# bupt-cist/vqa-playground-pytorch

Measured on AMD Instinct MI355X. Metric: VQA samples/sec (fwd+bwd), CoR2 batch 512, 36x2048 regions, higher is better.
Workload: dtype f32

## Files before the change

### vqa_playground_pytorch_amd/csrc/gemm_f32_split.hpp

```cpp
#pragma once
#include <type_traits>

#include "gemm_f32_rt.hpp"

namespace vqa {
namespace sp {

using rt::f32x4;
using rt::ldg16;
using rt::make_rsrc;
using rt::rsrc_t;
typedef uint32_t u32x4 __attribute__((ext_vector_type(4)));

constexpr int kThreads = 256;
constexpr int kChunk = 32;
constexpr int kPackedChunkBytes = 3 * 1024;

typedef float f32x2 __attribute__((ext_vector_type(2)));
typedef __bf16 bf16x2 __attribute__((ext_vector_type(2)));
__device__ __forceinline__ uint32_t opaque(uint32_t v) {
  asm("" : "+v"(v));
  return v;
}
__device__ __forceinline__ uint32_t pack2(f32x2 v) { return __builtin_bit_cast(uint32_t, __builtin_convertvector(v, bf16x2)); }
template <bool DOT>
__device__ __forceinline__ f32x2 residual(f32x2 x, uint32_t p) {
  if constexpr (DOT) {
    const bf16x2 pv = __builtin_bit_cast(bf16x2, p);
    const bf16x2 m0 = __builtin_bit_cast(bf16x2, opaque(0x0000BF80u)), m1 = __builtin_bit_cast(bf16x2, opaque(0xBF800000u));
    return f32x2{__builtin_amdgcn_fdot2_f32_bf16(pv, m0, x[0], false), __builtin_amdgcn_fdot2_f32_bf16(pv, m1, x[1], false)};
  } else {
    const f32x2 w = {bf16_lo(p), bf16_hi(p)};
    return x - w;
  }
}
template <bool DOT>
__device__ __forceinline__ void split_pair(f32x2 x, uint32_t& p0, uint32_t& p1, uint32_t& p2) {
  p0 = opaque(pack2(x));
  const f32x2 r = residual<DOT>(x, p0);
  p1 = opaque(pack2(r));
  const f32x2 t = residual<DOT>(r, p1);
  p2 = pack2(t);
}
struct Planes {
  u32x4 p[3];
};
template <bool DOT = true>
__device__ __forceinline__ void split8(const f32x4& lo, const f32x4& hi, Planes& o) {
  uint32_t w[3][4];
  split_pair<DOT>(__builtin_shufflevector(lo, lo, 0, 1), w[0][0], w[1][0], w[2][0]);
  split_pair<DOT>(__builtin_shufflevector(lo, lo, 2, 3), w[0][1], w[1][1], w[2][1]);
  split_pair<DOT>(__builtin_shufflevector(hi, hi, 0, 1), w[0][2], w[1][2], w[2][2]);
  split_pair<DOT>(__builtin_shufflevector(hi, hi, 2, 3), w[0][3], w[1][3], w[2][3]);
#pragma unroll
  for (int q = 0; q < 3; ++q) o.p[q] = u32x4{w[q][0], w[q][1], w[q][2], w[q][3]};
}
__device__ __forceinline__ f32x4 mfma_bf16(const u32x4& a, const u32x4& b, const f32x4& c) {
  return __builtin_amdgcn_mfma_f32_16x16x32_bf16(__builtin_bit_cast(bf16x8, a), __builtin_bit_cast(bf16x8, b), c, 0, 0, 0);
}

__device__ __forceinline__ uint32_t abs_bits_max(const f32x4& v) {
  const u32x4 b = __builtin_bit_cast(u32x4, v) & 0x7FFFFFFFu;
  return max(max(b[0], b[1]), max(b[2], b[3]));
}
__device__ __forceinline__ bool any_nonfinite(const f32x4& v) { return abs_bits_max(v) >= 0x7F800000u; }
__device__ __forceinline__ bool nonfinite(float v) { return (__float_as_uint(v) & 0x7FFFFFFFu) >= 0x7F800000u; }

template <bool DOT = false>
__global__ __launch_bounds__(256) void split_pack_kernel(const float* __restrict__ w, int ldw, int N, int K,
                                                         u32x4* __restrict__ out) {
  const int chunks = K / kChunk;
  const long t = (long)blockIdx.x * 256 + threadIdx.x;
  const int nblocks = (N + 15) / 16;
  if (t >= (long)nblocks * chunks * 64) return;
  const int lane = (int)(t & 63), r = lane & 15, g = lane >> 4;
  const long bc = t >> 6;
  const int c = (int)(bc % chunks), n = (int)(bc / chunks) * 16 + r;
  f32x4 lo = f32x4{0.f, 0.f, 0.f, 0.f}, hi = lo;
  if (n < N) {
    const float* src = w + (size_t)n * ldw + c * kChunk + 4 * g;
    lo = *reinterpret_cast<const f32x4*>(src);
    hi = *reinterpret_cast<const f32x4*>(src + 16);
  }
  Planes pl;
  split8<DOT>(lo, hi, pl);
  u32x4* dst = out + (size_t)bc * 192 + lane;
  dst[0] = pl.p[0];
  dst[64] = pl.p[1];
  dst[128] = pl.p[2];
}
__host__ __device__ inline size_t packed_bytes(int N, int K) { return (size_t)((N + 15) / 16) * (K / kChunk) * kPackedChunkBytes; }

struct NtArgs {
  const float* A;
  const u32x4* Bp;
  int lda;
  int M, N, K;
  int tiles_n;
  const float* Bf = nullptr;
  int ldb = 0;
  const float* T = nullptr;
  const float* C2 = nullptr;
  int rps = 0;
};
__host__ __device__ inline int rel_samples(int BM, int rps) { return (BM - 1) / rps + 2; }
__host__ __device__ inline size_t rel_lds_bytes(int BM, int rps, int K) { return (size_t)rel_samples(BM, rps) * 2 * K * 4; }
template <bool DROP>
__device__ __forceinline__ float nt_repair(const float* A, int lda, const float* Bf, int ldb, int K, int row, int col, uint32_t key,
                                           const float* T = nullptr, const float* C2 = nullptr, int rps = 1) {
  const float* a = A + (size_t)row * lda;
  const float* b = Bf + (size_t)col * ldb;
  float s = 0.f;
  for (int k = 0; k < K; ++k) {
    float x = a[k];
    if (T != nullptr) x = fmaf(C2[(size_t)(row / rps) * K + k], x, T[(size_t)(row / rps) * K + k]);
    if constexpr (DROP) {
      const uint32_t e = (uint32_t)row * (uint32_t)K + (uint32_t)k;
      x = ((mask_word32(e >> 5, key) >> (e & 31u)) & 1u) != 0u ? x : 0.f;
    }
    s = fmaf(x, b[k], s);
  }
  return s;
}

template <int RB, int CB, bool DROP, int TUNE, int NR, bool REL = false>
__device__ __forceinline__ void nt_accumulate(const NtArgs& p, const DropCfg& dc, size_t a_bytes, int m0, int n0, int c_lo, int c_hi,
                                              f32x4 (&acc)[RB][CB], const char* rel_lds = nullptr, int rel_s0 = 0) {
  static_assert((2 * RB) % NR == 0 && NR >= 2 && NR <= 2 * RB, "the ring must divide a pair of chunks");
  const int lane = threadIdx.x & 63, r = lane & 15, g = lane >> 4;
  const int chunks = p.K / kChunk;
  uint32_t offA[RB], offB[CB], wordA[RB];
  uint32_t offT[REL ? RB : 1];
#pragma unroll
  for (int i = 0; i < RB; ++i) {
    const int row = min(m0 + 16 * i + r, p.M - 1);
    offA[i] = ((uint32_t)row * (uint32_t)p.lda + 4u * g) * 4u;
    wordA[i] = ((uint32_t)row * (uint32_t)p.K) >> 5;
    if constexpr (REL) offT[i] = ((uint32_t)(row / p.rps - rel_s0) * 2u * (uint32_t)p.K + 4u * g) * 4u;
  }
#pragma unroll
  for (int j = 0; j < CB; ++j) {
    const int blk = min((n0 >> 4) + j, (p.N + 15) / 16 - 1);
    offB[j] = (uint32_t)blk * (uint32_t)chunks * (uint32_t)kPackedChunkBytes + 16u * lane;
  }
  const rsrc_t Ab = make_rsrc(p.A, a_bytes);
  const rsrc_t Bb = make_rsrc(p.Bp, packed_bytes(p.N, p.K));
  const uint32_t key = DROP ? drop_key(dc) : 0u;

  struct ARaw {
    f32x4 lo, hi;
  };
  auto loadA = [&](ARaw& a, int i, int c) {
    const uint32_t so = (uint32_t)c * 128u;
    constexpr int AUX = (TUNE & 128) ? 2 : 0;
    a.lo = __builtin_bit_cast(f32x4, __builtin_amdgcn_raw_buffer_load_b128(Ab, (int)offA[i], (int)so, AUX));
    a.hi = __builtin_bit_cast(f32x4, __builtin_amdgcn_raw_buffer_load_b128(Ab, (int)(offA[i] + 64u), (int)so, AUX));
  };
  auto loadB = [&](Planes(&b)[CB], int c) {
    const uint32_t so = (uint32_t)c * (uint32_t)kPackedChunkBytes;
#pragma unroll
    for (int j = 0; j < CB; ++j)
#pragma unroll
      for (int q = 0; q < 3; ++q)
        b[j].p[q] = __builtin_bit_cast(u32x4, __builtin_amdgcn_raw_buffer_load_b128(Bb, (int)(offB[j] + 1024u * q), (int)so, 0));
  };
  struct TC {
    f32x4 tlo, thi, clo, chi;
  };
  TC tc[REL ? 2 : 1];
  auto loadTC = [&](TC& o, int i, int c) {
    if constexpr (REL) {
      const char* base = rel_lds + offT[i] + (uint32_t)c * 128u;
      o.tlo = *reinterpret_cast<const f32x4*>(base);
      o.thi = *reinterpret_cast<const f32x4*>(base + 64);
      o.clo = *reinterpret_cast<const f32x4*>(base + (size_t)p.K * 4);
      o.chi = *reinterpret_cast<const f32x4*>(base + (size_t)p.K * 4 + 64);
    }
  };
  auto prepare = [&](const ARaw& a, Planes& pl, int i, int c, int n = 0) {
    if constexpr ((TUNE & 1) != 0) {
      pl.p[0] = __builtin_bit_cast(u32x4, a.lo);
      pl.p[1] = __builtin_bit_cast(u32x4, a.hi);
      pl.p[2] = __builtin_bit_cast(u32x4, a.lo);
    } else {
      ARaw m = a;
      if constexpr (REL) {
        const TC& q = tc[n & 1];
        m.lo = __builtin_elementwise_fma(q.clo, m.lo, q.tlo);
        m.hi = __builtin_elementwise_fma(q.chi, m.hi, q.thi);
      }
      if constexpr (DROP) {
        const uint32_t w = mask_word32(wordA[i] + (uint32_t)c, key);
        rt::keep4_bits(m.lo, w >> (4u * g));
        rt::keep4_bits(m.hi, w >> (4u * g + 16u));
      }
      split8<(TUNE & 64) != 0>(m.lo, m.hi, pl);
    }
  };
  auto mfma_row = [&](const Planes& a, const Planes(&b)[CB], int i) {
    constexpr int PA[6] = {0, 0, 1, 1, 0, 2}, PB[6] = {0, 1, 0, 1, 2, 0};
#pragma unroll
    for (int q = 0; q < 6; ++q)
#pragma unroll
      for (int j = 0; j < CB; ++j) acc[i][j] = mfma_bf16(a.p[PA[q]], b[j].p[PB[q]], acc[i][j]);
  };

  ARaw a[NR];
  Planes b0[CB], b1[CB], pl[2];
  auto fetch = [&](int n, int c_pair) {
    const int c = min(c_pair + n / RB, c_hi - 1);
    loadA(a[n % NR], n % RB, c);
  };
  auto loadB1 = [&](Planes(&b)[CB], int idx, int c) {
    b[idx / 3].p[idx % 3] = __builtin_bit_cast(u32x4, __builtin_amdgcn_raw_buffer_load_b128(
        Bb, (int)(offB[idx / 3] + 1024u * (idx % 3)), (int)((uint32_t)c * (uint32_t)kPackedChunkBytes), 0));
  };
  auto chunk = [&](Planes(&b)[CB], Planes(&bn)[CB], int c_pair, auto parity) {
    constexpr int P = decltype(parity)::value;
    constexpr int LB = (3 * CB + RB - 1) / RB;
    const int cb = min(c_pair + P + 1, c_hi - 1);
#pragma unroll
    for (int i = 0; i < RB; ++i) {
      const int n = P * RB + i;
      prepare(a[(n + 1) % NR], pl[(n + 1) & 1], (n + 1) % RB, min(c_pair + (n + 1) / RB, c_hi - 1), n + 1);
      if constexpr (REL) loadTC(tc[n & 1], (n + 2) % RB, min(c_pair + (n + 2) / RB, c_hi - 1));
      if constexpr ((TUNE & 2) == 0) fetch(n + 1 + NR, c_pair);
      int nb = 0;
      if constexpr ((TUNE & 32) == 0) {
#pragma unroll
        for (int idx = i * LB; idx < (i + 1) * LB && idx < 3 * CB; ++idx, ++nb) loadB1(bn, idx, cb);
      }
      mfma_row(pl[n & 1], b, i);
      constexpr int NM = 6 * CB;
      constexpr int VPM = ((TUNE >> 2) & 3) != 0 ? ((TUNE >> 2) & 3) : 2;
      const int nl = nb + ((TUNE & 2) == 0 ? 2 : 0);
      const int per = nl > 0 ? NM / nl : NM;
#pragma unroll
      for (int m = 0; m < NM; ++m) {
        __builtin_amdgcn_sched_group_barrier(0x008, 1, 0);
        if (REL && m < 4) __builtin_amdgcn_sched_group_barrier(0x100, 1, 0);
        __builtin_amdgcn_sched_group_barrier(0x002, VPM, 0);
        if (nl > 0 && m % per == per - 1 && m / per < nl) __builtin_amdgcn_sched_group_barrier(0x020, 1, 0);
      }
      __builtin_amdgcn_sched_barrier(0);
    }
  };
  if (c_lo < c_hi) {
    loadB(b0, c_lo);
#pragma unroll
    for (int n = 0; n < NR; ++n) fetch(n, c_lo);
    if constexpr (REL) {
      loadTC(tc[0], 0, c_lo);
      loadTC(tc[1], 1 % RB, min(c_lo + 1 / RB, c_hi - 1));
    }
    prepare(a[0], pl[0], 0, c_lo, 0);
    fetch(NR, c_lo);
    __builtin_amdgcn_sched_barrier(0);
    for (int c = c_lo; c < c_hi; c += 2) {
      chunk(b0, b1, c, std::integral_constant<int, 0>{});
      chunk(b1, b0, c, std::integral_constant<int, 1>{});
    }
  }

}

template <int RB, int CB, int NW, bool DROP, int TUNE>
__device__ __forceinline__ void nt_accumulate_shared(const NtArgs& p, const DropCfg& dc, size_t a_bytes, int m0, int n0, int c_lo,
                                                     int c_hi, int wave, char* lds_bytes, f32x4 (&acc)[RB][CB]) {
  constexpr int MINE = (RB + NW - 1) / NW;
  const int lane = threadIdx.x & 63, r = lane & 15, g = lane >> 4;
  const int chunks = p.K / kChunk;
  u32x4* const lds = reinterpret_cast<u32x4*>(lds_bytes);
  uint32_t offA[MINE], offB[CB], wordA[MINE];
#pragma unroll
  for (int k = 0; k < MINE; ++k) {
    const int i = min(wave + NW * k, RB - 1);
    const int row = min(m0 + 16 * i + r, p.M - 1);
    offA[k] = ((uint32_t)row * (uint32_t)p.lda + 4u * g) * 4u;
    wordA[k] = ((uint32_t)row * (uint32_t)p.K) >> 5;
  }
  const uint32_t key = DROP ? drop_key(dc) : 0u;
#pragma unroll
  for (int j = 0; j < CB; ++j) {
    const int blk = min((n0 >> 4) + j, (p.N + 15) / 16 - 1);
    offB[j] = (uint32_t)blk * (uint32_t)chunks * (uint32_t)kPackedChunkBytes + 16u * lane;
  }
  const rsrc_t Ab = make_rsrc(p.A, a_bytes);
  const rsrc_t Bb = make_rsrc(p.Bp, packed_bytes(p.N, p.K));
  struct ARaw {
    f32x4 lo, hi;
  };
  ARaw raw0[MINE], raw1[MINE];
  Planes b0[CB], b1[CB], xp[2];
  auto loadA = [&](ARaw(&raw)[MINE], int c) {
    const uint32_t so = (uint32_t)min(c, c_hi - 1) * 128u;
#pragma unroll
    for (int k = 0; k < MINE; ++k) {
      raw[k].lo = ldg16(Ab, offA[k], so);
      raw[k].hi = ldg16(Ab, offA[k] + 64u, so);
    }
  };
  auto loadB1 = [&](Planes(&b)[CB], int idx, int c) {
    b[idx / 3].p[idx % 3] = __builtin_bit_cast(u32x4, __builtin_amdgcn_raw_buffer_load_b128(
        Bb, (int)(offB[idx / 3] + 1024u * (idx % 3)), (int)((uint32_t)min(c, c_hi - 1) * (uint32_t)kPackedChunkBytes), 0));
  };
  auto produce = [&](const ARaw& a, int k, int buf, int c) {
    if (wave + NW * k < RB) {
      Planes pl;
      ARaw m = a;
      if constexpr (DROP) {
        const uint32_t w = mask_word32(wordA[k] + (uint32_t)min(c, c_hi - 1), key);
        rt::keep4_bits(m.lo, w >> (4u * g));
        rt::keep4_bits(m.hi, w >> (4u * g + 16u));
      }
      split8<false>(m.lo, m.hi, pl);
      u32x4* dst = lds + ((size_t)(buf * RB + wave + NW * k) * 3) * 64 + lane;
#pragma unroll
      for (int q = 0; q < 3; ++q) dst[64 * q] = pl.p[q];
    }
  };
  auto fetch = [&](Planes& o, int i, int buf) {
    const u32x4* src = lds + ((size_t)(buf * RB + i) * 3) * 64 + lane;
#pragma unroll
    for (int q = 0; q < 3; ++q) o.p[q] = src[64 * q];
  };
  auto mfma_row = [&](const Planes& a, const Planes(&b)[CB], int i) {
    constexpr int PA[6] = {0, 0, 1, 1, 0, 2}, PB[6] = {0, 1, 0, 1, 2, 0};
#pragma unroll
    for (int q = 0; q < 6; ++q)
#pragma unroll
      for (int j = 0; j < CB; ++j) acc[i][j] = mfma_bf16(a.p[PA[q]], b[j].p[PB[q]], acc[i][j]);
  };
  auto chunk = [&](Planes(&b)[CB], Planes(&bn)[CB], ARaw(&rn)[MINE], ARaw(&rf)[MINE], int c, auto parity) {
    constexpr int P = decltype(parity)::value;
    constexpr int LB = (3 * CB + RB - 2) / (RB - 1);
    int bidx = 0, pk = 0;
#pragma unroll
    for (int i = 0; i < RB; ++i) {
      const int n = P * RB + i;
      if (i == RB - 1) __syncthreads();
      if (i + 1 < RB) fetch(xp[(n + 1) & 1], i + 1, P);
      else fetch(xp[(n + 1) & 1], 0, P ^ 1);
      if (i == 0) loadA(rf, c + 2);
      if (i >= 1 && pk < MINE && i < RB - 1) {
        produce(rn[pk], pk, P ^ 1, c + 1);
        ++pk;
      }
      int nl = 0;
      if (i < RB - 1) {
#pragma unroll
        for (int k = 0; k < LB; ++k)
          if (bidx < 3 * CB) {
            loadB1(bn, bidx, c + 1);
            ++bidx;
            ++nl;
          }
      }
      mfma_row(xp[n & 1], b, i);
      constexpr int NM = 6 * CB;
#pragma unroll
      for (int m = 0; m < NM; ++m) {
        __builtin_amdgcn_sched_group_barrier(0x008, 1, 0);
        if (m < 3) __builtin_amdgcn_sched_group_barrier(0x100, 1, 0);
        __builtin_amdgcn_sched_group_barrier(0x002, 2, 0);
        if (m >= 4 && m < 4 + 2 * (2 * MINE + LB) && (m & 1) == 0) __builtin_amdgcn_sched_group_barrier(0x020, 1, 0);
        if (m >= NM - 6 && (m & 1) == 0) __builtin_amdgcn_sched_group_barrier(0x200, 1, 0);
      }
      __builtin_amdgcn_sched_barrier(0);
    }
  };
  static_assert(MINE <= RB - 2, "a wave's row blocks are produced in the regions 1 .. RB - 2");
  if (c_lo < c_hi) {
#pragma unroll
    for (int idx = 0; idx < 3 * CB; ++idx) loadB1(b0, idx, c_lo);
    loadA(raw0, c_lo);
    loadA(raw1, c_lo + 1);
#pragma unroll
    for (int k = 0; k < MINE; ++k) produce(raw0[k], k, 0, c_lo);
    __syncthreads();
    fetch(xp[0], 0, 0);
    __builtin_amdgcn_sched_barrier(0);
    for (int c = c_lo; c < c_hi; c += 2) {
      chunk(b0, b1, raw1, raw0, c, std::integral_constant<int, 0>{});
      chunk(b1, b0, raw0, raw1, c + 1, std::integral_constant<int, 1>{});
    }
  }
}

template <int RB, int WN, int WK, bool SHARE_A>
constexpr size_t nt_lds_bytes(size_t reduction_bytes) {
  return SHARE_A ? (reduction_bytes > (size_t)WK * 2 * RB * 3 * 1024 ? reduction_bytes : (size_t)WK * 2 * RB * 3 * 1024) : reduction_bytes;
}
template <int RB, int CB, int WM, int WN, int WK, bool DROP, class Epi, int TUNE = 0, int NR = RB, bool SHARE_A = false, bool REL = false>
__global__ __launch_bounds__(kThreads, 1) void gemm_nt_kernel(NtArgs p, DropCfg dc, Epi epi) {
  using S = rt::NtShape<RB, CB, WM, WN, WK>;
  static_assert(!SHARE_A || WM == 1, "SHARE_A: the waves of a K range share their rows");
  static_assert(!(REL && SHARE_A), "REL is built on the per-wave split");
  const int lane = threadIdx.x & 63, r = lane & 15, g = lane >> 4;
  const int wave = __builtin_amdgcn_readfirstlane(threadIdx.x >> 6);
  const int wk = wave / (WM * WN), wmn = wave % (WM * WN), wm = wmn / WN, wn = wmn % WN;
  const int tile = xcd_remap(blockIdx.x, gridDim.x);
  const int tiles_m = gridDim.x / p.tiles_n;
  const int tm = (TUNE & 16) ? tile % tiles_m : tile / p.tiles_n, tn = (TUNE & 16) ? tile / tiles_m : tile % p.tiles_n;
  const int m0 = tm * S::BM + wm * (16 * RB);
  const int n0 = tn * S::BN + wn * (16 * CB);
  const int chunks = p.K / kChunk;

  f32x4 acc[RB][CB];
#pragma unroll
  for (int i = 0; i < RB; ++i)
#pragma unroll
    for (int j = 0; j < CB; ++j) acc[i][j] = f32x4{0.f, 0.f, 0.f, 0.f};
  const int per = ((chunks + WK - 1) / WK + 1) & ~1;
  const int c_lo = min(chunks, wk * per), c_hi = min(chunks, c_lo + per);

  if constexpr (SHARE_A) {
    extern __shared__ __attribute__((aligned(16))) char sp_smem[];
    nt_accumulate_shared<RB, CB, WN, DROP, TUNE>(p, dc, ((size_t)(p.M - 1) * p.lda + p.K) * 4, m0, n0, c_lo, c_hi, wn,
                                                 sp_smem + (size_t)wk * 2 * RB * 3 * 1024, acc);
    __syncthreads();
  } else if constexpr (REL) {
    extern __shared__ __attribute__((aligned(16))) char sp_smem[];
    const int s0 = (tm * S::BM) / p.rps;
    const int ns = (min(p.M, (tm + 1) * S::BM) - 1) / p.rps - s0 + 1;
    const int k4 = p.K / 4;
    const int total = ns * 2 * k4, iters = (total + kThreads - 1) / kThreads;
    for (int it = 0; it < iters; ++it) {
      const int idx = min(it * kThreads + (int)threadIdx.x, total - 1);
      const int s = idx / (2 * k4), rem = idx - s * 2 * k4, which = rem / k4, k = rem - which * k4;
      const float* src = (which == 0 ? p.T : p.C2) + (size_t)(s0 + s) * p.K + 4 * k;
      reinterpret_cast<f32x4*>(sp_smem)[idx] = *reinterpret_cast<const f32x4*>(src);
    }
    __syncthreads();
    nt_accumulate<RB, CB, DROP, TUNE, NR, true>(p, dc, ((size_t)(p.M - 1) * p.lda + p.K) * 4, m0, n0, c_lo, c_hi, acc, sp_smem, s0);
    __syncthreads();
  } else {
    nt_accumulate<RB, CB, DROP, TUNE, NR>(p, dc, ((size_t)(p.M - 1) * p.lda + p.K) * 4, m0, n0, c_lo, c_hi, acc);
  }

  uint64_t bad = 0;
  auto finish = [&](int blk, f32x4 v) {
    const int i = blk / CB, j = blk % CB;
    const int col = n0 + 16 * j + r;
    if (any_nonfinite(v)) bad |= 1ull << blk;
    if (col < p.N) {
#pragma unroll
      for (int t = 0; t < 4; ++t) {
        const int row = m0 + 16 * i + 4 * g + t;
        if (row < p.M) epi(row, col, v[t]);
      }
    }
  };
  if constexpr (WK == 2) {
    extern __shared__ __attribute__((aligned(16))) char sp_smem[];
    f32x4* red = reinterpret_cast<f32x4*>(sp_smem);
    f32x4* out_box = red + (size_t)((wmn * 2 + wk) * S::HALF) * 64 + lane;
    const f32x4* in_box = red + (size_t)((wmn * 2 + (wk ^ 1)) * S::HALF) * 64 + lane;
    if (wk == 0) {
#pragma unroll
      for (int blk = S::HALF; blk < S::NB; ++blk) out_box[(blk - S::HALF) * 64] = acc[blk / CB][blk % CB];
    } else {
#pragma unroll
      for (int blk = 0; blk < S::HALF; ++blk) out_box[blk * 64] = acc[blk / CB][blk % CB];
    }
    __syncthreads();
    if (wk == 0) {
#pragma unroll
      for (int blk = 0; blk < S::HALF; ++blk) finish(blk, acc[blk / CB][blk % CB] + in_box[blk * 64]);
    } else {
#pragma unroll
      for (int blk = S::HALF; blk < S::NB; ++blk) finish(blk, acc[blk / CB][blk % CB] + in_box[(blk - S::HALF) * 64]);
    }
  } else {
#pragma unroll
    for (int blk = 0; blk < S::NB; ++blk) finish(blk, acc[blk / CB][blk % CB]);
  }
  static_assert(S::NB <= 64, "one bit per accumulator block");
  if (p.Bf != nullptr && bad != 0) {
    const uint32_t key = DROP ? drop_key(dc) : 0u;
    for (int blk = 0; blk < S::NB; ++blk) {
      if (((bad >> blk) & 1ull) == 0) continue;
      const int col = n0 + 16 * (blk % CB) + r;
      if (col >= p.N) continue;
      for (int t = 0; t < 4; ++t) {
        const int row = m0 + 16 * (blk / CB) + 4 * g + t;
        if (row < p.M) epi(row, col, nt_repair<DROP>(p.A, p.lda, p.Bf, p.ldb, p.K, row, col, key, REL ? p.T : nullptr, p.C2, REL ? p.rps : 1));
      }
    }
  }
}


struct TnArgs {
  const u32x4* Gp;
  const float* X;
  float* slab;
  int ldx;
  int M, N1, N2;
  int nblocks;
  int cps;
  int tiles1, tiles2;
  const float* Gf = nullptr;
  const float* Yf = nullptr;
  int ldg = 0;
  const float* T = nullptr;
  const float* C2 = nullptr;
  int rps = 0;
  uint32_t rps_magic = 0;
};
inline uint32_t rps_magic_of(int rps) { return (uint32_t)((1ull << 32) / (uint64_t)rps + 1ull); }
template <int NA, int SPN, bool DROP>
__device__ __forceinline__ void tn_store(const TnArgs& p, const DropCfg& dc, const f32x4 (&acc)[NA][4 * SPN], int slab, int b1, int n2_0,
                                         int r, int g) {
  float* out = p.slab + (size_t)slab * p.N1 * p.N2;
  uint64_t bad = 0;
  static_assert(NA * SPN * 4 <= 64, "one bit per 16-byte store");
#pragma unroll
  for (int i = 0; i < NA; ++i)
#pragma unroll
    for (int q = 0; q < SPN; ++q) {
      const int col = n2_0 + 64 * q + 4 * r;
#pragma unroll
      for (int t = 0; t < 4; ++t) {
        const int n1 = 16 * (b1 + i) + 4 * g + t;
        const f32x4 v = f32x4{acc[i][4 * q][t], acc[i][4 * q + 1][t], acc[i][4 * q + 2][t], acc[i][4 * q + 3][t]};
        if (b1 + i < p.nblocks && n1 < p.N1 && col + 3 < p.N2) {
          *reinterpret_cast<f32x4*>(out + (size_t)n1 * p.N2 + col) = v;
          if (any_nonfinite(v)) bad |= 1ull << ((i * SPN + q) * 4 + t);
        }
      }
    }
  if (p.Gf != nullptr && bad != 0) {
    const uint32_t key = DROP ? drop_key(dc) : 0u;
    const int m_lo = slab * p.cps * kChunk, m_hi = min(p.M, m_lo + p.cps * kChunk);
    for (int k = 0; k < NA * SPN * 4; ++k) {
      if (((bad >> k) & 1ull) == 0) continue;
      const int t = k & 3, q = (k >> 2) % SPN, i = (k >> 2) / SPN;
      const int n1 = 16 * (b1 + i) + 4 * g + t, col = n2_0 + 64 * q + 4 * r;
      f32x4 sum = f32x4{0.f, 0.f, 0.f, 0.f};
      for (int m = m_lo; m < m_hi; ++m) {
        float gv = p.Gf[(size_t)m * p.ldg + n1];
        if (p.Yf != nullptr) gv = p.Yf[(size_t)m * p.ldg + n1] > 0.f ? gv : 0.f;
        f32x4 x = *reinterpret_cast<const f32x4*>(p.X + (size_t)m * p.ldx + col);
        if (p.T != nullptr) {
          const size_t at = (size_t)(m / p.rps) * p.N2 + col;
          x = __builtin_elementwise_fma(*reinterpret_cast<const f32x4*>(p.C2 + at), x, *reinterpret_cast<const f32x4*>(p.T + at));
        }
        if constexpr (DROP) {
          const uint32_t e = (uint32_t)m * (uint32_t)p.N2 + (uint32_t)col;
          const uint32_t w = mask_word32(e >> 5, key) >> (e & 31u);
#pragma unroll
          for (int c = 0; c < 4; ++c) x[c] = ((w >> c) & 1u) != 0u ? x[c] : 0.f;
        }
#pragma unroll
        for (int c = 0; c < 4; ++c) sum[c] = fmaf(gv, x[c], sum[c]);
      }
      *reinterpret_cast<f32x4*>(out + (size_t)n1 * p.N2 + col) = sum;
    }
  }
}
struct TnPlan {
  int slabs, cps;
};
inline TnPlan tn_plan(int M, int want_slabs) {
  const int chunks = (M + kChunk - 1) / kChunk;
  int S = want_slabs < 1 ? 1 : want_slabs;
  if (S > (chunks + 1) / 2) S = (chunks + 1) / 2;
  int cps = ((chunks + S - 1) / S + 1) & ~1;
  S = (chunks + cps - 1) / cps;
  return {S, cps};
}
__host__ __device__ inline size_t packed_tn_bytes(int slabs, int cps, int N1) {
  return (size_t)slabs * cps * ((N1 + 15) / 16) * kPackedChunkBytes;
}

constexpr int kPackParts = 36;
template <bool GATE, bool WRITE_GZ>
__global__ __launch_bounds__(256) void pack_tn_kernel(const float* __restrict__ gy, const float* __restrict__ y, int ld, int M,
                                                      int N1_all, int nblocks, int cps, u32x4* __restrict__ out,
                                                      float* __restrict__ dbslab, float* __restrict__ gz, int nblk_total) {
  extern __shared__ __attribute__((aligned(16))) float pk_tile[];
  const int pitch = 16 * nblocks + 1;
  const int lane = threadIdx.x & 63, r = lane & 15, g = lane >> 4, wave = threadIdx.x >> 6;
  const int slab = blockIdx.x / kPackParts, part = blockIdx.x % kPackParts;
  const int per = (cps + kPackParts - 1) / kPackParts;
  const int lo = part * per, hi = min(cps, lo + per);
  const int blk0 = blockIdx.y * nblocks, c0 = 16 * blk0;
  const int N1 = min(N1_all - c0, 16 * nblocks);
  gy += c0;
  if (GATE) y += c0;
  if (WRITE_GZ) gz += c0;
  const int pairs = N1 / 2;
  float colsum[8];
#pragma unroll
  for (int k = 0; k < 8; ++k) colsum[k] = 0.f;
  for (int cc = lo; cc < hi; ++cc) {
    const int c = slab * cps + cc;
    const int m0 = c * kChunk;
#pragma unroll 2
    for (int row = wave; row < 32; row += 4) {
      const int m = m0 + row;
      for (int cp = lane; cp < pairs; cp += 64) {
        float2 v = make_float2(0.f, 0.f);
        if (m < M) {
          v = *reinterpret_cast<const float2*>(gy + (size_t)m * ld + 2 * cp);
          if constexpr (GATE) {
            const float2 yy = *reinterpret_cast<const float2*>(y + (size_t)m * ld + 2 * cp);
            v.x = yy.x > 0.f ? v.x : 0.f;
            v.y = yy.y > 0.f ? v.y : 0.f;
          }
          if constexpr (WRITE_GZ) *reinterpret_cast<float2*>(gz + (size_t)m * ld + 2 * cp) = v;
        }
        pk_tile[row * pitch + 2 * cp] = v.x;
        pk_tile[row * pitch + 2 * cp + 1] = v.y;
      }
    }
    __syncthreads();
#pragma unroll
    for (int k = 0; k < 8; ++k) {
      const int blk = wave + 4 * k;
      if (blk < nblocks && blk0 + blk < nblk_total) {
        const int col = 16 * blk + r;
        float v[8];
#pragma unroll
        for (int j = 0; j < 8; ++j) v[j] = col < N1 ? pk_tile[(8 * g + j) * pitch + col] : 0.f;
        uint32_t w[3][4];
#pragma unroll
        for (int jj = 0; jj < 4; ++jj) {
          split_pair<false>(f32x2{v[2 * jj], v[2 * jj + 1]}, w[0][jj], w[1][jj], w[2][jj]);
          colsum[k] += v[2 * jj] + v[2 * jj + 1];
        }
        u32x4* dst = out + ((size_t)c * nblk_total + blk0 + blk) * 192 + lane;
#pragma unroll
        for (int q = 0; q < 3; ++q) dst[64 * q] = u32x4{w[q][0], w[q][1], w[q][2], w[q][3]};
      }
    }
    __syncthreads();
  }
  if (dbslab != nullptr) {
#pragma unroll
    for (int k = 0; k < 8; ++k) {
      float sum = colsum[k];
      sum += __shfl_xor(sum, 16);
      sum += __shfl_xor(sum, 32);
      const int col = 16 * (wave + 4 * k) + r;
      if (g == 0 && wave + 4 * k < nblocks && col < N1) dbslab[(size_t)blockIdx.x * N1_all + c0 + col] = sum;
    }
  }
}
inline size_t pack_tn_lds_bytes(int nblocks) { return (size_t)32 * (16 * nblocks + 1) * sizeof(float); }
constexpr int kPackMaxBlocks = 30;

template <int NA, int SPN, bool DROP, int TUNE = 0>
__global__ __launch_bounds__(kThreads, 1) void gemm_tn_kernel(TnArgs p, DropCfg dc) {
  constexpr int NBX = 4 * SPN;
  static_assert(NBX % 2 == 0, "plane sets alternate per block");
  const int lane = threadIdx.x & 63, r = lane & 15, g = lane >> 4;
  const int wave = __builtin_amdgcn_readfirstlane(threadIdx.x >> 6);
  const int bid = xcd_remap(blockIdx.x, gridDim.x);
  const int tiles = p.tiles1 * p.tiles2;
  const int slab = bid / tiles, tile = bid % tiles;
  const int t2 = tile % p.tiles2, t1 = tile / p.tiles2;
  const int b1 = (t1 * 4 + wave) * NA;
  const int n2_0 = t2 * (64 * SPN);
  const int c_lo = slab * p.cps, c_hi = c_lo + p.cps;

  uint32_t offX[8], offG[NA];
#pragma unroll
  for (int j = 0; j < 8; ++j)
    offX[j] = ((uint32_t)(8 * g + j) * (uint32_t)p.ldx + (uint32_t)min(n2_0 + 4 * r, p.N2 - 4)) * 4u;
#pragma unroll
  for (int i = 0; i < NA; ++i) offG[i] = (uint32_t)min(b1 + i, p.nblocks - 1) * (uint32_t)kPackedChunkBytes + 16u * lane;
  const rsrc_t Xb = make_rsrc(p.X, ((size_t)(p.M - 1) * p.ldx + p.N2) * 4);
  const rsrc_t Gb = make_rsrc(p.Gp, (size_t)gridDim.x / tiles * p.cps * p.nblocks * kPackedChunkBytes);
  const uint32_t key = DROP ? drop_key(dc) : 0u;
  const uint32_t chunk_stride_x = 32u * (uint32_t)p.ldx * 4u, chunk_stride_g = (uint32_t)p.nblocks * (uint32_t)kPackedChunkBytes;

  f32x4 acc[NA][NBX];
#pragma unroll
  for (int i = 0; i < NA; ++i)
#pragma unroll
    for (int b = 0; b < NBX; ++b) acc[i][b] = f32x4{0.f, 0.f, 0.f, 0.f};

  f32x4 xr[SPN][8];
  Planes g0[NA], g1[NA], pl[2];
  auto loadX = [&](int q, int c) {
    const uint32_t so = (uint32_t)c * chunk_stride_x;
// ... 316 lines not shown
```

### vqa_playground_pytorch_amd/csrc/relation_dgrad_split.hip

```cpp
#include <cstdlib>

#include "gemm_f32_split.hpp"

namespace vqa {
namespace {

constexpr int kRegions = 36, kRB = 9, kSamples = 4, kBM = 16 * kRB;

struct RelSplitArgs {
  const float* gz;
  const sp::u32x4* wp;
  const float* v;
  float* d_t;
  float* d_c2;
  int B, M, L, D;
  int Kp;
  int tiles_n;
  int v_nt = 0;
  int col_major = 0;
  const float* wf;
};

__global__ __launch_bounds__(256) void pack_wt_kernel(const float* __restrict__ w, int L, int D, int chunks,
                                                      sp::u32x4* __restrict__ out) {
  const long t = (long)blockIdx.x * 256 + threadIdx.x;
  if (t >= (long)(D / 16) * chunks * 64) return;
  const int lane = (int)(t & 63), r = lane & 15, g = lane >> 4;
  const long bc = t >> 6;
  const int c = (int)(bc % chunks), cb = (int)(bc / chunks);
  const int d = 64 * (cb / 4) + 4 * r + (cb % 4);
  float v[8];
#pragma unroll
  for (int j = 0; j < 8; ++j) {
    const int l = 32 * c + 4 * g + (j & 3) + 16 * (j >> 2);
    v[j] = l < L ? w[(size_t)l * D + d] : 0.f;
  }
  uint32_t pw[3][4];
#pragma unroll
  for (int jj = 0; jj < 4; ++jj) sp::split_pair<false>(sp::f32x2{v[2 * jj], v[2 * jj + 1]}, pw[0][jj], pw[1][jj], pw[2][jj]);
  sp::u32x4* dst = out + (size_t)bc * 192 + lane;
#pragma unroll
  for (int q = 0; q < 3; ++q) dst[64 * q] = sp::u32x4{pw[q][0], pw[q][1], pw[q][2], pw[q][3]};
}

constexpr int kSharedLds = 2 * kRB * 3 * 1024;
template <bool SHARED, int TUNE = 0>
__global__ __launch_bounds__(sp::kThreads, 1) void relation_dgrad_split_kernel(RelSplitArgs p, DropCfg dc) {
  using rt::f32x4;
  const int lane = threadIdx.x & 63, r = lane & 15, g = lane >> 4;
  const int wave = __builtin_amdgcn_readfirstlane(threadIdx.x >> 6);
  const int tile = xcd_remap(blockIdx.x, gridDim.x);
  const int tiles_m_ = gridDim.x / p.tiles_n;
  const int m0 = (p.col_major ? tile % tiles_m_ : tile / p.tiles_n) * kBM;
  const int n0 = (p.col_major ? tile / tiles_m_ : tile % p.tiles_n) * 256 + 64 * wave;
  if (!SHARED && n0 >= p.D) return;
  const int M = p.M, D = p.D;

  const rt::rsrc_t Vb = rt::make_rsrc(p.v, (size_t)M * D * 4);
  f32x4 acc[kRB][4];
#pragma unroll
  for (int i = 0; i < kRB; ++i)
#pragma unroll
    for (int e = 0; e < 4; ++e) acc[i][e] = f32x4{0.f, 0.f, 0.f, 0.f};
  {
    const sp::NtArgs a{p.gz, p.wp, p.L, M, D, p.Kp, p.tiles_n};
    if constexpr ((TUNE & 1) != 0) {
      acc[0][0] = f32x4{(float)m0, (float)n0, 1.f, 2.f};
    } else if constexpr (SHARED) {
      extern __shared__ __attribute__((aligned(16))) char rd_smem[];
      sp::nt_accumulate_shared<kRB, 4, 4, false, 0>(a, dc, (size_t)M * p.L * 4, m0, n0, 0, p.Kp / sp::kChunk, wave, rd_smem, acc);
    } else {
      sp::nt_accumulate<kRB, 4, false, 0, 3>(a, dc, (size_t)M * p.L * 4, m0, n0, 0, p.Kp / sp::kChunk, acc);
    }
  }

  if constexpr (TUNE == 0) {
    uint32_t top = 0;
#pragma unroll
    for (int i = 0; i < kRB; ++i)
#pragma unroll
      for (int e = 0; e < 4; ++e) top = max(top, sp::abs_bits_max(acc[i][e]));
    if (top >= 0x7F800000u) {
#pragma unroll 1
      for (int it = 0; it < 4 * kRB; ++it) {
        const float* grow = p.gz + (size_t)min(m0 + 16 * (it >> 2) + 4 * g + (it & 3), M - 1) * p.L;
        const float* wcol = p.wf + n0 + 4 * r;
        f32x4 s = f32x4{0.f, 0.f, 0.f, 0.f};
        for (int l = 0; l < p.L; ++l) {
          const float gv = grow[l];
          const f32x4 wv = *reinterpret_cast<const f32x4*>(wcol + (size_t)l * D);
#pragma unroll
          for (int e = 0; e < 4; ++e) s[e] = fmaf(gv, wv[e], s[e]);
        }
#pragma unroll
        for (int i = 0; i < kRB; ++i)
#pragma unroll
          for (int t = 0; t < 4; ++t)
#pragma unroll
            for (int e = 0; e < 4; ++e) acc[i][e][t] = it == 4 * i + t ? s[e] : acc[i][e][t];
      }
    }
  }

  if constexpr ((TUNE & 4) != 0) {
    f32x4 sum = f32x4{0.f, 0.f, 0.f, 0.f};
#pragma unroll
    for (int i = 0; i < kRB; ++i)
#pragma unroll
      for (int e = 0; e < 4; ++e) sum += acc[i][e];
    if (g == 0) *reinterpret_cast<f32x4*>(p.d_t + (size_t)(m0 / kRegions) * D + n0 + 4 * r) = sum;
    return;
  }
  auto vt = [&](int i, int t) -> f32x4 {
    if constexpr ((TUNE & 2) != 0) return f32x4{1.f, 1.f, 1.f, 1.f};
    const int row = min(m0 + 16 * i + 4 * g + t, M - 1);
    const uint32_t off = (uint32_t)(n0 + 4 * r) * 4u + (uint32_t)row * (uint32_t)D * 4u;
    if (p.v_nt) return __builtin_bit_cast(f32x4, __builtin_amdgcn_raw_buffer_load_b128(Vb, (int)off, 0, 2));
    return rt::ldg16(Vb, off, 0u);
  };
  const uint32_t key = dc.p8 > 0 ? drop_key(dc) : 0u;
  if (m0 + kBM > M) {
#pragma unroll
    for (int i = 0; i < kRB; ++i)
#pragma unroll
      for (int t = 0; t < 4; ++t)
        if (m0 + 16 * i + 4 * g + t >= M) {
#pragma unroll
          for (int e = 0; e < 4; ++e) acc[i][e][t] = 0.f;
        }
  }
  f32x4 st[kSamples], sc[kSamples];
#pragma unroll
  for (int s = 0; s < kSamples; ++s) st[s] = sc[s] = f32x4{0.f, 0.f, 0.f, 0.f};
  auto reduce = [&](auto mode) {
    constexpr int MODE = decltype(mode)::value;
#pragma unroll
    for (int i = 0; i < kRB; ++i) {
      f32x4 xt = f32x4{0.f, 0.f, 0.f, 0.f}, xc = f32x4{0.f, 0.f, 0.f, 0.f};
#pragma unroll
      for (int t = 0; t < 4; ++t) {
        f32x4 x = f32x4{acc[i][0][t], acc[i][1][t], acc[i][2][t], acc[i][3][t]};
        if constexpr (MODE != 0) {
          const int m = min(m0 + 16 * i + 4 * g + t, M - 1);
          const uint32_t e = (uint32_t)m * (uint32_t)D + (uint32_t)(n0 + 4 * r);
          if constexpr (MODE == 1) {
            const uint32_t w = mask_word32(e >> 5, key) >> (e & 31u);
#pragma unroll
            for (int c = 0; c < 4; ++c) {
              const float xe = x[c];
              x[c] = __uint_as_float(__float_as_uint(xe) & (0u - ((w >> c) & 1u)));
            }
          } else {
            const uint32_t w = mask_word32(e >> 2, key);
            x *= f32x4{(w & 255u) >= dc.p8 ? dc.scale : 0.f, ((w >> 8) & 255u) >= dc.p8 ? dc.scale : 0.f,
                       ((w >> 16) & 255u) >= dc.p8 ? dc.scale : 0.f, (w >> 24) >= dc.p8 ? dc.scale : 0.f};
          }
        }
        xt += x;
        xc += x * vt(i, t);
      }
      constexpr int kGroups = kRegions / 4;
      const int s_lo = (4 * i) / kGroups, s_hi = (4 * i + 3) / kGroups;
      if (s_lo == s_hi) {
        st[s_lo] += xt;
        sc[s_lo] += xc;
      } else {
        const bool hi = (4 * i + g) / kGroups == s_hi;
        const f32x4 z = f32x4{0.f, 0.f, 0.f, 0.f};
        st[s_lo] += hi ? z : xt;
        sc[s_lo] += hi ? z : xc;
        st[s_hi] += hi ? xt : z;
        sc[s_hi] += hi ? xc : z;
      }
    }
  };
  if (dc.p8 == 0) reduce(std::integral_constant<int, 0>{});
  else if (dc.p8 == kDropHalf) reduce(std::integral_constant<int, 1>{});
  else reduce(std::integral_constant<int, 2>{});
  const float post = dc.p8 == kDropHalf ? 2.f : 1.f;
  const int b0 = m0 / kRegions;
#pragma unroll
  for (int s = 0; s < kSamples; ++s) {
    f32x4 a, b;
#pragma unroll
    for (int e = 0; e < 4; ++e) {
      a[e] = rows_sum(st[s][e]) * post;
      b[e] = rows_sum(sc[s][e]) * post;
    }
    if (g == 0 && b0 + s < p.B) {
      *reinterpret_cast<f32x4*>(p.d_t + (size_t)(b0 + s) * D + n0 + 4 * r) = a;
      *reinterpret_cast<f32x4*>(p.d_c2 + (size_t)(b0 + s) * D + n0 + 4 * r) = b;
    }
  }
}

int padded_k(int L) { return (((L + sp::kChunk - 1) / sp::kChunk + 1) & ~1) * sp::kChunk; }

}
}

using namespace vqa;

extern "C" int vqa_relation_projection_dgrad_split_supported(int B, int N, int D, int L) {
  return N == kRegions && B >= 1 && D % 64 == 0 && D >= 64 && L >= 32 && L % 2 == 0 && (size_t)B * N * D * 4 < (1ull << 32) &&
         sp::packed_bytes(D, padded_k(L)) < (1ull << 32) && (size_t)B * N * L * 4 < (1ull << 32);
}

extern "C" size_t vqa_relation_projection_dgrad_split_workspace_bytes(int D, int L) {
  return (sp::packed_bytes(D, padded_k(L)) + 255) & ~(size_t)255;
}

extern "C" int vqa_relation_projection_dgrad_split(const float* gz, const float* w, const float* v, float* d_t, float* d_c2,
                                                   void* workspace, size_t workspace_bytes, float p_drop, uint64_t seed,
                                                   const uint64_t* seed_ptr, int B, int N, int D, int L, vqa_stream_t stream) {
  VQA_REQUIRE(gz && w && v && d_t && d_c2 && workspace, VQA_E_BADARG, "relation_projection_dgrad_split: null pointer");
  VQA_REQUIRE(p_drop >= 0.f && p_drop < 1.f, VQA_E_BADARG, "relation_projection_dgrad_split: p_drop=%f outside [0,1)", (double)p_drop);
  VQA_REQUIRE(B > 0 && N > 0 && D > 0 && L > 0, VQA_E_BADARG, "relation_projection_dgrad_split: bad sizes B=%d N=%d D=%d L=%d", B, N, D, L);
  VQA_REQUIRE(vqa_relation_projection_dgrad_split_supported(B, N, D, L), VQA_E_UNSUPPORTED,
              "relation_projection_dgrad_split: needs N = 36 regions, D %% 64 == 0, even L >= 32 (N=%d D=%d L=%d)", N, D, L);
  VQA_REQUIRE(aligned(w, 16) && aligned(v, 16) && aligned(d_t, 16) && aligned(d_c2, 16) && aligned(gz, 8) && aligned(workspace, 16),
              VQA_E_UNSUPPORTED, "relation_projection_dgrad_split: w, v, d_t, d_c2, workspace must be 16-byte aligned, gz 8-byte");
  VQA_REQUIRE(workspace_bytes >= vqa_relation_projection_dgrad_split_workspace_bytes(D, L), VQA_E_BADARG,
              "relation_projection_dgrad_split: workspace too small");
  hipStream_t s = static_cast<hipStream_t>(stream);
  const int Kp = padded_k(L), chunks = Kp / sp::kChunk;
  sp::u32x4* wp = static_cast<sp::u32x4*>(workspace);
  {
    const long threads = (long)(D / 16) * chunks * 64;
    VQA_LAUNCH(pack_wt_kernel, dim3((unsigned)((threads + 255) / 256)), dim3(256), 0, s, w, L, D, chunks, wp);
  }
  RelSplitArgs a{};
  a.gz = gz;
  a.wp = wp;
  a.v = v;
  a.d_t = d_t;
  a.d_c2 = d_c2;
  a.B = B;
  a.M = B * N;
  a.L = L;
  a.D = D;
  a.Kp = Kp;
  a.tiles_n = (D + 255) / 256;
  a.wf = w;
  const int tiles_m = (a.M + kBM - 1) / kBM;
  const DropCfg dc = make_drop(p_drop, seed, seed_ptr);
  a.col_major = vqa::option_is("VQA_SPLIT_DGRAD_ORDER", 'c') ? 1 : 0;
  a.v_nt = vqa::option_is("VQA_SPLIT_DGRAD_VNT", '1') ? 1 : 0;
  const int tune = vqa::option("VQA_SPLIT_DGRAD_TUNE") ? std::atoi(vqa::option("VQA_SPLIT_DGRAD_TUNE")) : 0;
  const dim3 grid_((unsigned)(tiles_m * a.tiles_n));
  if (tune == 1 && D % 256 == 0) VQA_LAUNCH((relation_dgrad_split_kernel<true, 1>), grid_, dim3(sp::kThreads), kSharedLds, s, a, dc);
  else if (tune == 2 && D % 256 == 0) VQA_LAUNCH((relation_dgrad_split_kernel<true, 2>), grid_, dim3(sp::kThreads), kSharedLds, s, a, dc);
  else if (tune == 4 && D % 256 == 0) VQA_LAUNCH((relation_dgrad_split_kernel<true, 4>), grid_, dim3(sp::kThreads), kSharedLds, s, a, dc);
  else if (tune == 5 && D % 256 == 0) VQA_LAUNCH((relation_dgrad_split_kernel<true, 5>), grid_, dim3(sp::kThreads), kSharedLds, s, a, dc);
  else if (D % 256 == 0 && !vqa::option_is("VQA_SPLIT_DGRAD_SHARED", '0'))
    VQA_LAUNCH(relation_dgrad_split_kernel<true>, dim3((unsigned)(tiles_m * a.tiles_n)), dim3(sp::kThreads), kSharedLds, s, a, dc);
  else
    VQA_LAUNCH(relation_dgrad_split_kernel<false>, dim3((unsigned)(tiles_m * a.tiles_n)), dim3(sp::kThreads), 0, s, a, dc);
  return check_launch("relation_projection_dgrad_split");
}
```

Measured before the change: 260,900.

## Prefetch v tile into registers during last GEMM chunk via scheduling hook

Adds a hook mechanism to the NT GEMM accumulate loops so the relation dgrad kernel can issue its loads of v inside the final K-chunk, interleaved with the MFMAs. The epilogue then reads the prefetched registers instead of loading v after the GEMM finishes. The goal is to hide the epilogue's global-memory latency behind matrix math. In exchange it holds a kRB x 4 f32x4 register array live across the final chunk, which raises register pressure and could cause spills. It also peels the last loop iteration.

Result: no change. 262,000 (median of 6 runs) (+0.4%).

```diff
diff --git a/vqa_playground_pytorch_amd/csrc/gemm_f32_split.hpp b/vqa_playground_pytorch_amd/csrc/gemm_f32_split.hpp
--- a/vqa_playground_pytorch_amd/csrc/gemm_f32_split.hpp
+++ b/vqa_playground_pytorch_amd/csrc/gemm_f32_split.hpp
@@ -103,6 +103,18 @@
   const float* C2 = nullptr;
   int rps = 0;
 };
+struct NtNoHook {
+  static constexpr int kLoads = 0;
+  __device__ __forceinline__ void operator()(int) const {}
+};
+template <int N, class F>
+struct NtHook {
+  static constexpr int kLoads = N;
+  F f;
+  __device__ __forceinline__ void operator()(int i) const { f(i); }
+};
+template <int N, class F>
+__device__ __forceinline__ NtHook<N, F> nt_hook(F f) { return NtHook<N, F>{f}; }
 __host__ __device__ inline int rel_samples(int BM, int rps) { return (BM - 1) / rps + 2; }
 __host__ __device__ inline size_t rel_lds_bytes(int BM, int rps, int K) { return (size_t)rel_samples(BM, rps) * 2 * K * 4; }
 template <bool DROP>
@@ -123,9 +135,10 @@
   return s;
 }
 
-template <int RB, int CB, bool DROP, int TUNE, int NR, bool REL = false>
+template <int RB, int CB, bool DROP, int TUNE, int NR, bool REL = false, class Hook = NtNoHook>
 __device__ __forceinline__ void nt_accumulate(const NtArgs& p, const DropCfg& dc, size_t a_bytes, int m0, int n0, int c_lo, int c_hi,
-                                              f32x4 (&acc)[RB][CB], const char* rel_lds = nullptr, int rel_s0 = 0) {
+                                              f32x4 (&acc)[RB][CB], const char* rel_lds = nullptr, int rel_s0 = 0,
+                                              const Hook& hook = Hook{}) {
   static_assert((2 * RB) % NR == 0 && NR >= 2 && NR <= 2 * RB, "the ring must divide a pair of chunks");
   const int lane = threadIdx.x & 63, r = lane & 15, g = lane >> 4;
   const int chunks = p.K / kChunk;
@@ -215,8 +228,9 @@
     b[idx / 3].p[idx % 3] = __builtin_bit_cast(u32x4, __builtin_amdgcn_raw_buffer_load_b128(
         Bb, (int)(offB[idx / 3] + 1024u * (idx % 3)), (int)((uint32_t)c * (uint32_t)kPackedChunkBytes), 0));
   };
-  auto chunk = [&](Planes(&b)[CB], Planes(&bn)[CB], int c_pair, auto parity) {
+  auto chunk = [&](Planes(&b)[CB], Planes(&bn)[CB], int c_pair, auto parity, auto hooked) {
     constexpr int P = decltype(parity)::value;
+    constexpr int NH = decltype(hooked)::value ? Hook::kLoads : 0;
     constexpr int LB = (3 * CB + RB - 1) / RB;
     const int cb = min(c_pair + P + 1, c_hi - 1);
 #pragma unroll
@@ -230,10 +244,11 @@
 #pragma unroll
         for (int idx = i * LB; idx < (i + 1) * LB && idx < 3 * CB; ++idx, ++nb) loadB1(bn, idx, cb);
       }
+      if constexpr (NH > 0) hook(i);
       mfma_row(pl[n & 1], b, i);
       constexpr int NM = 6 * CB;
       constexpr int VPM = ((TUNE >> 2) & 3) != 0 ? ((TUNE >> 2) & 3) : 2;
-      const int nl = nb + ((TUNE & 2) == 0 ? 2 : 0);
+      const int nl = nb + ((TUNE & 2) == 0 ? 2 : 0) + NH;
       const int per = nl > 0 ? NM / nl : NM;
 #pragma unroll
       for (int m = 0; m < NM; ++m) {
@@ -256,17 +271,28 @@
     prepare(a[0], pl[0], 0, c_lo, 0);
     fetch(NR, c_lo);
     __builtin_amdgcn_sched_barrier(0);
-    for (int c = c_lo; c < c_hi; c += 2) {
-      chunk(b0, b1, c, std::integral_constant<int, 0>{});
-      chunk(b1, b0, c, std::integral_constant<int, 1>{});
-    }
-  }
-
-}
-
-template <int RB, int CB, int NW, bool DROP, int TUNE>
+    if constexpr (Hook::kLoads == 0) {
+      for (int c = c_lo; c < c_hi; c += 2) {
+        chunk(b0, b1, c, std::integral_constant<int, 0>{}, std::false_type{});
+        chunk(b1, b0, c, std::integral_constant<int, 1>{}, std::false_type{});
+      }
+    } else {
+      int c = c_lo;
+      for (; c + 2 < c_hi; c += 2) {
+        chunk(b0, b1, c, std::integral_constant<int, 0>{}, std::false_type{});
+        chunk(b1, b0, c, std::integral_constant<int, 1>{}, std::false_type{});
+      }
+      chunk(b0, b1, c, std::integral_constant<int, 0>{}, std::false_type{});
+      chunk(b1, b0, c, std::integral_constant<int, 1>{}, std::true_type{});
+    }
+  }
+
+}
+
+template <int RB, int CB, int NW, bool DROP, int TUNE, class Hook = NtNoHook>
 __device__ __forceinline__ void nt_accumulate_shared(const NtArgs& p, const DropCfg& dc, size_t a_bytes, int m0, int n0, int c_lo,
-                                                     int c_hi, int wave, char* lds_bytes, f32x4 (&acc)[RB][CB]) {
+                                                     int c_hi, int wave, char* lds_bytes, f32x4 (&acc)[RB][CB],
+                                                     const Hook& hook = Hook{}) {
   constexpr int MINE = (RB + NW - 1) / NW;
   const int lane = threadIdx.x & 63, r = lane & 15, g = lane >> 4;
   const int chunks = p.K / kChunk;
@@ -331,8 +357,9 @@
 #pragma unroll
       for (int j = 0; j < CB; ++j) acc[i][j] = mfma_bf16(a.p[PA[q]], b[j].p[PB[q]], acc[i][j]);
   };
-  auto chunk = [&](Planes(&b)[CB], Planes(&bn)[CB], ARaw(&rn)[MINE], ARaw(&rf)[MINE], int c, auto parity) {
+  auto chunk = [&](Planes(&b)[CB], Planes(&bn)[CB], ARaw(&rn)[MINE], ARaw(&rf)[MINE], int c, auto parity, auto hooked) {
     constexpr int P = decltype(parity)::value;
+    constexpr int NH = decltype(hooked)::value ? Hook::kLoads : 0;
     constexpr int LB = (3 * CB + RB - 2) / (RB - 1);
     int bidx = 0, pk = 0;
 #pragma unroll
@@ -356,6 +383,7 @@
             ++nl;
           }
       }
+      if constexpr (NH > 0) hook(i);
       mfma_row(xp[n & 1], b, i);
       constexpr int NM = 6 * CB;
 #pragma unroll
@@ -363,7 +391,7 @@
         __builtin_amdgcn_sched_group_barrier(0x008, 1, 0);
         if (m < 3) __builtin_amdgcn_sched_group_barrier(0x100, 1, 0);
         __builtin_amdgcn_sched_group_barrier(0x002, 2, 0);
-        if (m >= 4 && m < 4 + 2 * (2 * MINE + LB) && (m & 1) == 0) __builtin_amdgcn_sched_group_barrier(0x020, 1, 0);
+        if (m >= 4 && m < 4 + 2 * (2 * MINE + LB + NH) && (m & 1) == 0) __builtin_amdgcn_sched_group_barrier(0x020, 1, 0);
         if (m >= NM - 6 && (m & 1) == 0) __builtin_amdgcn_sched_group_barrier(0x200, 1, 0);
       }
       __builtin_amdgcn_sched_barrier(0);
@@ -380,9 +408,19 @@
     __syncthreads();
     fetch(xp[0], 0, 0);
     __builtin_amdgcn_sched_barrier(0);
-    for (int c = c_lo; c < c_hi; c += 2) {
-      chunk(b0, b1, raw1, raw0, c, std::integral_constant<int, 0>{});
-      chunk(b1, b0, raw0, raw1, c + 1, std::integral_constant<int, 1>{});
+    if constexpr (Hook::kLoads == 0) {
+      for (int c = c_lo; c < c_hi; c += 2) {
+        chunk(b0, b1, raw1, raw0, c, std::integral_constant<int, 0>{}, std::false_type{});
+        chunk(b1, b0, raw0, raw1, c + 1, std::integral_constant<int, 1>{}, std::false_type{});
+      }
+    } else {
+      int c = c_lo;
+      for (; c + 2 < c_hi; c += 2) {
+        chunk(b0, b1, raw1, raw0, c, std::integral_constant<int, 0>{}, std::false_type{});
+        chunk(b1, b0, raw0, raw1, c + 1, std::integral_constant<int, 1>{}, std::false_type{});
+      }
+      chunk(b0, b1, raw1, raw0, c, std::integral_constant<int, 0>{}, std::false_type{});
+      chunk(b1, b0, raw0, raw1, c + 1, std::integral_constant<int, 1>{}, std::true_type{});
     }
   }
 }
diff --git a/vqa_playground_pytorch_amd/csrc/relation_dgrad_split.hip b/vqa_playground_pytorch_amd/csrc/relation_dgrad_split.hip
--- a/vqa_playground_pytorch_amd/csrc/relation_dgrad_split.hip
+++ b/vqa_playground_pytorch_amd/csrc/relation_dgrad_split.hip
@@ -44,7 +44,7 @@
 }
 
 constexpr int kSharedLds = 2 * kRB * 3 * 1024;
-template <bool SHARED, int TUNE = 0>
+template <bool SHARED, int TUNE = 0, bool VNT = false>
 __global__ __launch_bounds__(sp::kThreads, 1) void relation_dgrad_split_kernel(RelSplitArgs p, DropCfg dc) {
   using rt::f32x4;
   const int lane = threadIdx.x & 63, r = lane & 15, g = lane >> 4;
@@ -57,6 +57,22 @@
   const int M = p.M, D = p.D;
 
   const rt::rsrc_t Vb = rt::make_rsrc(p.v, (size_t)M * D * 4);
+  auto vt = [&](int i, int t) -> f32x4 {
+    if constexpr ((TUNE & 2) != 0) return f32x4{1.f, 1.f, 1.f, 1.f};
+    const int row = min(m0 + 16 * i + 4 * g + t, M - 1);
+    const uint32_t off = (uint32_t)(n0 + 4 * r) * 4u + (uint32_t)row * (uint32_t)D * 4u;
+    return __builtin_bit_cast(f32x4, __builtin_amdgcn_raw_buffer_load_b128(Vb, (int)off, 0, VNT ? 2 : 0));
+  };
+  constexpr int kVFirst = SHARED ? 4 : 0, kVPer = SHARED ? 8 : 4;
+  static_assert((kRB - kVFirst) * kVPer >= 4 * kRB, "every load of v has a row block to go out in");
+  f32x4 vpre[kRB][4];
+  const auto vhook = sp::nt_hook<kVPer>([&](int i) {
+#pragma unroll
+    for (int k = 0; k < kVPer; ++k) {
+      const int idx = (i - kVFirst) * kVPer + k;
+      if (idx >= 0 && idx < 4 * kRB) vpre[idx >> 2][idx & 3] = vt(idx >> 2, idx & 3);
+    }
+  });
   f32x4 acc[kRB][4];
 #pragma unroll
   for (int i = 0; i < kRB; ++i)
@@ -66,11 +82,14 @@
     const sp::NtArgs a{p.gz, p.wp, p.L, M, D, p.Kp, p.tiles_n};
     if constexpr ((TUNE & 1) != 0) {
       acc[0][0] = f32x4{(float)m0, (float)n0, 1.f, 2.f};
+#pragma unroll
+      for (int i = 0; i < kRB; ++i) vhook(i);
     } else if constexpr (SHARED) {
       extern __shared__ __attribute__((aligned(16))) char rd_smem[];
-      sp::nt_accumulate_shared<kRB, 4, 4, false, 0>(a, dc, (size_t)M * p.L * 4, m0, n0, 0, p.Kp / sp::kChunk, wave, rd_smem, acc);
+      sp::nt_accumulate_shared<kRB, 4, 4, false, 0>(a, dc, (size_t)M * p.L * 4, m0, n0, 0, p.Kp / sp::kChunk, wave, rd_smem, acc,
+                                                    vhook);
     } else {
-      sp::nt_accumulate<kRB, 4, false, 0, 3>(a, dc, (size_t)M * p.L * 4, m0, n0, 0, p.Kp / sp::kChunk, acc);
+      sp::nt_accumulate<kRB, 4, false, 0, 3, false>(a, dc, (size_t)M * p.L * 4, m0, n0, 0, p.Kp / sp::kChunk, acc, nullptr, 0, vhook);
     }
   }
 
@@ -111,13 +130,6 @@
     if (g == 0) *reinterpret_cast<f32x4*>(p.d_t + (size_t)(m0 / kRegions) * D + n0 + 4 * r) = sum;
     return;
   }
-  auto vt = [&](int i, int t) -> f32x4 {
-    if constexpr ((TUNE & 2) != 0) return f32x4{1.f, 1.f, 1.f, 1.f};
-    const int row = min(m0 + 16 * i + 4 * g + t, M - 1);
-    const uint32_t off = (uint32_t)(n0 + 4 * r) * 4u + (uint32_t)row * (uint32_t)D * 4u;
-    if (p.v_nt) return __builtin_bit_cast(f32x4, __builtin_amdgcn_raw_buffer_load_b128(Vb, (int)off, 0, 2));
-    return rt::ldg16(Vb, off, 0u);
-  };
   const uint32_t key = dc.p8 > 0 ? drop_key(dc) : 0u;
   if (m0 + kBM > M) {
 #pragma unroll
@@ -157,7 +169,7 @@
           }
         }
         xt += x;
-        xc += x * vt(i, t);
+        xc += x * vpre[i][t];
       }
       constexpr int kGroups = kRegions / 4;
       const int s_lo = (4 * i) / kGroups, s_hi = (4 * i + 3) / kGroups;
@@ -252,9 +264,12 @@
   else if (tune == 2 && D % 256 == 0) VQA_LAUNCH((relation_dgrad_split_kernel<true, 2>), grid_, dim3(sp::kThreads), kSharedLds, s, a, dc);
   else if (tune == 4 && D % 256 == 0) VQA_LAUNCH((relation_dgrad_split_kernel<true, 4>), grid_, dim3(sp::kThreads), kSharedLds, s, a, dc);
   else if (tune == 5 && D % 256 == 0) VQA_LAUNCH((relation_dgrad_split_kernel<true, 5>), grid_, dim3(sp::kThreads), kSharedLds, s, a, dc);
-  else if (D % 256 == 0 && !vqa::option_is("VQA_SPLIT_DGRAD_SHARED", '0'))
-    VQA_LAUNCH(relation_dgrad_split_kernel<true>, dim3((unsigned)(tiles_m * a.tiles_n)), dim3(sp::kThreads), kSharedLds, s, a, dc);
-  else
-    VQA_LAUNCH(relation_dgrad_split_kernel<false>, dim3((unsigned)(tiles_m * a.tiles_n)), dim3(sp::kThreads), 0, s, a, dc);
+  else if (D % 256 == 0 && !vqa::option_is("VQA_SPLIT_DGRAD_SHARED", '0')) {
+    if (a.v_nt) VQA_LAUNCH((relation_dgrad_split_kernel<true, 0, true>), grid_, dim3(sp::kThreads), kSharedLds, s, a, dc);
+    else VQA_LAUNCH(relation_dgrad_split_kernel<true>, grid_, dim3(sp::kThreads), kSharedLds, s, a, dc);
+  } else {
+    if (a.v_nt) VQA_LAUNCH((relation_dgrad_split_kernel<false, 0, true>), grid_, dim3(sp::kThreads), 0, s, a, dc);
+    else VQA_LAUNCH(relation_dgrad_split_kernel<false>, grid_, dim3(sp::kThreads), 0, s, a, dc);
+  }
   return check_launch("relation_projection_dgrad_split");
 }
```
